# oneam/h264bsd

Measured on AMD Instinct MI355X. Metric: 1080p macroblocks/s, higher is better.
Workload: dtype u8; 1 GPU; 256 concurrent copies of test_1920x1080.h264 per GPU (73 pictures x 8160 MB), kernel-only replay from HBM-resident frame jobs, inter+intra reconstruction + in-loop deblocking; streams_per_gpu=256, parallelism=streams/1, stream_groups=1, row_bands=library default (engine.hip TailConfig)

## Files before the change

h264bsd_amd/csrc/engine.hip:

```cpp
#include <hip/hip_runtime.h>
#include <stdio.h>
#include <stdlib.h>
#include <string.h>
#include <deque>
#include <memory>
#include <mutex>
#include <vector>
#include <algorithm>
#include "kernels.hip.h"
#include "kernels/k_tensor_out.hip.h"
#include "kernels/k_tensor_aa.hip.h"
#include "kernels/k_tensor_roi.hip.h"
#include "kernels/k_tensor_remap.hip.h"
#include "kernels/k_motion.hip.h"
#include "kernels/region_common.hip.h"
#include "kernels/k_region_stats.hip.h"
#include "kernels/k_keep.hip.h"
#include "kernels/k_blend.hip.h"
#include "kernels/k_region_change.hip.h"
#include "kernels/k_region_shift.hip.h"
#include "kernels/k_cell_maps.hip.h"
#include "kernels/k_cell_boxes.hip.h"
#include "engine.h"
#include "hip_owned.h"
// ... 190 lines not shown
        Lane &l = lanes[i];
        if (g == 1 && i == 0) { l.st = e->stream; l.side = &e->side; }
        else { HIP_TRY(l.own_st.create()); l.st = l.own_st; }
        HIP_TRY(l.tail.create(hipEventDisableTiming));
        for (auto &ev : l.ring) HIP_TRY(ev.create(hipEventDisableTiming));
    }
    e->n_light = g; e->n_heavy = k;
    e->lanes.swap(lanes);
    return 0;
}

Engine *engine_get(int device = -1)
{
    if (device < 0) device = current_device();
    if (device >= MAX_DEVICES) return nullptr;
    std::lock_guard<std::mutex> lk(g_engine_mu);
    if (g_engines[device]) return g_engines[device];
    int n = 0;
    if (hipGetDeviceCount(&n) != hipSuccess || n <= 0 || device >= n) return nullptr;
    std::unique_ptr<Engine> e(new Engine());
    e->device = device;
    if (hipSetDevice(e->device) != hipSuccess || e->stream.create() != hipSuccess || e->inflight_done.create(hipEventDisableTiming) != hipSuccess ||
        ![&] {
            int lo = 0, hi = 0;
            const bool prio = hipDeviceGetStreamPriorityRange(&lo, &hi) == hipSuccess;
            return e->side.create(hi, prio);
        }() ||
        e->d_err.alloc(256) != hipSuccess || hipMemset(e->d_err, 0, 256) != hipSuccess || hipDeviceSynchronize() != hipSuccess ||
        e->h_err.alloc(64, true) != hipSuccess) return nullptr;
    e->h_err[0] = e->h_err[1] = 0;
    return g_engines[device] = e.release();
}

TailConfig g_tail;
std::mutex g_tail_mu;
TailConfig tail_config()
{
    std::lock_guard<std::mutex> lk(g_tail_mu);
    if (!g_tail.from_env) {
        g_tail.from_env = true;
        if (const char *cfg = getenv("H264BSDMI_TAIL")) {
            unsigned v[7] = { 0, 0, 0, 0, 0, 0, 0 };
            if (sscanf(cfg, "%u,%u,%u,%u,%u,%u,%u", &v[0], &v[1], &v[2], &v[3], &v[4], &v[5], &v[6]) >= 6) {
                g_tail.dbk_rows_light = v[0]; g_tail.dbk_rows_heavy = v[1]; g_tail.dbk_waves = v[2];
                g_tail.intra_rows_light = v[3]; g_tail.intra_rows_heavy = v[4]; g_tail.intra_waves = v[5];
                g_tail.dbk_chroma_waves = v[6];
            } else fprintf(stderr, "h264bsd-mi355x: H264BSDMI_TAIL=%s ignored (expected six or seven numbers)\n", cfg);
        }
        if (const char *cfg = getenv("H264BSDMI_BAND_BUDGET")) g_tail.band_budget = (uint32_t)strtoul(cfg, nullptr, 10);
        if (const char *cfg = getenv("H264BSDMI_HEAVY_BUDGET")) g_tail.heavy_budget = (uint32_t)strtoul(cfg, nullptr, 10);
    }
    return g_tail;
}
static uint16_t bands_for(uint32_t hmb, uint32_t rows)
{
    if (!rows || rows >= hmb) return 1;
    return (uint16_t)std::min<uint32_t>((hmb + rows - 1) / rows, 64u);
}

std::mutex g_ticket_mu;
auto *const g_tickets = new std::vector<std::pair<hipStream_t, DeviceMem<uint32_t>>>[MAX_DEVICES];
static uint32_t *tickets_for(hipStream_t st)
{
    int dev = 0;
    if (hipGetDevice(&dev) != hipSuccess || dev < 0 || dev >= MAX_DEVICES) return nullptr;
    std::lock_guard<std::mutex> lk(g_ticket_mu);
    for (auto &p : g_tickets[dev]) if (p.first == st) return p.second;
    DeviceMem<uint32_t> d;
    if (d.alloc(64) != hipSuccess || hipMemsetAsync(d, 0, 64, st) != hipSuccess) return nullptr;
    g_tickets[dev].emplace_back(st, std::move(d));
    return g_tickets[dev].back().second;
}
}
void tickets_release(hipStream_t st)
{
    std::lock_guard<std::mutex> lk(g_ticket_mu);
    for (int d = 0; d < MAX_DEVICES; d++)
        g_tickets[d].erase(std::remove_if(g_tickets[d].begin(), g_tickets[d].end(), [&](const auto &p) { return p.first == st; }), g_tickets[d].end());
}
namespace {
static void tickets_rezero(int dev)
{
    std::lock_guard<std::mutex> lk(g_ticket_mu);
    if (dev < 0 || dev >= MAX_DEVICES) return;
    for (auto &p : g_tickets[dev]) (void)hipMemsetAsync(p.second, 0, 64, p.first);
}


void make_desc(FrameDesc &d, const uint8_t *host_blob, const uint8_t *dev_blob, uint8_t *dev_frames, uint32_t frame_bytes,
               uint8_t *dev_dbk, TickShape *shape, uint32_t *dev_err)
{
    const FjHeader *h = reinterpret_cast<const FjHeader *>(host_blob);
    d.recs = reinterpret_cast<const FjMbRec *>(dev_blob + h->rec_off);
    d.mvx = reinterpret_cast<const int16_t *>(dev_blob + h->mvx_off);
    d.coefs = reinterpret_cast<const int16_t *>(dev_blob + h->coef_off);
    d.lvl = reinterpret_cast<const uint32_t *>(dev_blob + h->lvl_off);
    d.idx = reinterpret_cast<const uint16_t *>(dev_blob + h->idx_off);
    d.copy = reinterpret_cast<const FjCopy *>(dev_blob + h->copy_off);
    d.gen = reinterpret_cast<const FjGen *>(dev_blob + h->gen_off);
    d.n_copy = h->n_copy;
    d.n_gen = h->n_gen;
    d.n_gen_uni = h->n_gen_uniform;
    d.n_gen_quad = h->n_gen_quad;
    d.dbki = reinterpret_cast<const uint16_t *>(dev_blob + h->dbk_off);
    d.n_dbk = h->n_dbk;
    d.dbk = dev_dbk;
    d.cur = dev_frames + (size_t)h->cur_slot * frame_bytes;
    d.n_mbs = h->n_mbs;
    d.n_levels = h->n_intra_levels;
    d.wmb = h->width_mbs;
    d.wmb_magic = (uint32_t)(0x100000000ull / (h->width_mbs ? h->width_mbs : 1u)) + 1u;
    d.hmb = h->height_mbs;
    d.any_deblock = h->any_deblock;
    {
        const TailConfig tc = tail_config();
        const bool heavy = h->n_intra * 4u > h->n_mbs;
        d.heavy = heavy ? 1 : 0;
        d.dbk_bands = bands_for(h->height_mbs, heavy ? tc.dbk_rows_heavy : tc.dbk_rows_light);
        d.intra_bands = h->intra_down_deps ? 1 : bands_for(h->height_mbs, heavy ? tc.intra_rows_heavy : tc.intra_rows_light);
    }
    d.err = dev_err;
    d.conv_src = nullptr; d.conv_dst = nullptr; d.conv_fmt = 0; d.conv_pad = 0;
    for (uint32_t k = 0; k < FJ_MAX_SLOTS; k++) d.slot[k] = k < h->n_slots ? dev_frames + (size_t)k * frame_bytes : nullptr;
    if (shape) {
        shape->n_frames++;
        shape->max_mbs = std::max(shape->max_mbs, h->n_mbs);
        shape->max_copy = std::max(shape->max_copy, h->n_copy);
        shape->max_gen = std::max(shape->max_gen, h->n_gen);
        shape->max_gen_uni = std::max(shape->max_gen_uni, h->n_gen_uniform);
        shape->max_gen_quad = std::max(shape->max_gen_quad, h->n_gen_quad);
        shape->max_gen_rest = std::max(shape->max_gen_rest, h->n_gen - h->n_gen_uniform - h->n_gen_quad);
        shape->max_dbk = std::max(shape->max_dbk, h->n_dbk);
        shape->any_deblock |= h->any_deblock != 0;
        shape->max_levels = std::max(shape->max_levels, h->n_intra_levels);
        shape->max_w = std::max<uint32_t>(shape->max_w, h->width_mbs);
        shape->max_h = std::max<uint32_t>(shape->max_h, h->height_mbs);
        shape->any_tail |= h->n_intra_levels != 0 || h->any_deblock != 0;
        shape->n_heavy += d.heavy;
        if (h->any_deblock) (d.heavy ? shape->want_heavy : shape->want_light)[0] = std::max<uint32_t>((d.heavy ? shape->want_heavy : shape->want_light)[0], d.dbk_bands);
        if (h->n_intra_levels) (d.heavy ? shape->want_heavy : shape->want_light)[1] = std::max<uint32_t>((d.heavy ? shape->want_heavy : shape->want_light)[1], d.intra_bands);
        if (h->n_intra_levels && h->intra_down_deps) shape->intra_whole = true;
    }
}

struct TickTimers { Event ev[6]; Event sev[5]; bool on = false; bool copy_timed = false; unsigned mask = 31u; };

static void launch_kdbk(hipStream_t st, const FrameDesc *d_desc, const TickShape &s, uint32_t launches[5])
{
    hipLaunchKernelGGL(h264k::k_dbk, dim3((s.max_dbk + 64 * DBK_WG_WAVES - 1) / (64 * DBK_WG_WAVES), s.n_frames), dim3(64 * DBK_WG_WAVES), 0, st, d_desc);
    if (launches) launches[2]++;
}
template <int PATH> static void launch_inter(hipStream_t st, const FrameDesc *d_desc, uint32_t n_max, uint32_t n_frames)
{
    constexpr uint32_t per_wg = INTER_WG_WAVES * h264k::inter_per_wave<PATH>();
    if (n_max) hipLaunchKernelGGL(h264k::k_recon_inter<PATH>, dim3((n_max + per_wg - 1) / per_wg, n_frames), dim3(64 * INTER_WG_WAVES), 0, st, d_desc);
}
std::mutex g_tail_lds_mu;
size_t g_tail_lds[2][2][MAX_DEVICES] = {};
static int tail_prepare(hipStream_t st, int which, const BandPlan &bp, const void *fn, uint32_t **tickets)
{
    const bool banded = bp.bands > 1;
    *tickets = banded ? tickets_for(st) : nullptr;
    if (banded && !*tickets) return -1;
    int dev = 0;
    HIP_TRY(hipGetDevice(&dev));
    std::lock_guard<std::mutex> lk(g_tail_lds_mu);
    if (bp.lds > g_tail_lds[which][banded][dev]) {
        HIP_TRY(hipFuncSetAttribute(fn, hipFuncAttributeMaxDynamicSharedMemorySize, (int)bp.lds));
        g_tail_lds[which][banded][dev] = bp.lds;
    }
    return 0;
}

int launch_tick(hipStream_t st, const FrameDesc *d_desc, const TickShape &s, TickTimers *tt, uint32_t launches[5],
                unsigned stages = 7u, const SideLane *side = nullptr, unsigned long long *prof = nullptr)
{
    const bool timed = tt && tt->on;
    const unsigned tmask = timed ? tt->mask : 0u;
    auto boundary = [&](unsigned i) -> int {
        if ((((tmask << 1) | tmask) >> i) & 1u) HIP_TRY(hipEventRecord(tt->ev[i], st));
        return 0;
    };
    if (boundary(0)) return -1;
    const bool do_dbk = (stages & 4u) && s.any_deblock && s.max_dbk;
    const bool do_copy = (stages & 1u) && s.max_copy;
    const bool aside = side && side->stream && do_dbk;
    const bool copy_aside = aside && do_copy && side->copy_stream;
    if (tt) tt->copy_timed = false;
    auto launch_copy = [&](hipStream_t cs) {
        hipLaunchKernelGGL(h264k::k_copy, dim3(std::min<uint32_t>((s.max_copy + 3) / 4, COPY_WGS), s.n_frames), dim3(256), 0, cs, d_desc);
        if (launches) launches[0]++;
    };
    if (aside) {
        HIP_TRY(hipEventRecord(side->fork, st));
        HIP_TRY(hipStreamWaitEvent(side->stream, side->fork, 0));
        if (copy_aside) {
            const bool ctimed = timed && (tmask & 1u) && tt->sev[3] && tt->sev[4];
            if (tt) tt->copy_timed = ctimed;
            HIP_TRY(hipStreamWaitEvent(side->copy_stream, side->fork, 0));
            if (ctimed) HIP_TRY(hipEventRecord(tt->sev[3], side->copy_stream));
            launch_copy(side->copy_stream);
            if (ctimed) HIP_TRY(hipEventRecord(tt->sev[4], side->copy_stream));
            HIP_TRY(hipEventRecord(side->copy_join, side->copy_stream));
        }
        const bool dtimed = timed && (tmask & 4u);
        if (dtimed && tt->sev[1]) HIP_TRY(hipEventRecord(tt->sev[1], side->stream));
        launch_kdbk(side->stream, d_desc, s, launches);
        if (dtimed && tt->sev[2]) HIP_TRY(hipEventRecord(tt->sev[2], side->stream));
        HIP_TRY(hipEventRecord(side->join, side->stream));
    }
    if (do_copy && !copy_aside) launch_copy(st);
    if (boundary(1)) return -1;
    if ((stages & 1u) && s.max_gen) {
        launch_inter<0>(st, d_desc, s.max_gen_uni, s.n_frames);
        launch_inter<1>(st, d_desc, s.max_gen_quad, s.n_frames);
        launch_inter<2>(st, d_desc, s.max_gen_rest, s.n_frames);
        if (launches) launches[1]++;
    }
    if (boundary(2)) return -1;
    if (do_dbk && !aside) launch_kdbk(st, d_desc, s, launches);
    if (boundary(3)) return -1;
    const TailConfig tc = tail_config();
    if (copy_aside) HIP_TRY(hipStreamWaitEvent(st, side->copy_join, 0));
    if (s.max_levels && (stages & 2u)) {
        BandPlan bp;
        if (plan_bands(s, tc, 1, std::max<uint32_t>(1u, std::min<uint32_t>(tc.intra_waves, h264k::TAIL_WAVES)), h264k::intra_lds_bytes, false, bp)) {
            fprintf(stderr, "h264bsd-mi355x: picture of %u x %u macroblocks is too large for k_frame_intra\n", s.max_w, s.max_h); return -1;
        }
        uint32_t *tickets;
        if (tail_prepare(st, 1, bp, bp.bands > 1 ? (const void *)h264k::k_frame_intra<true> : (const void *)h264k::k_frame_intra<false>, &tickets)) return -1;
        if (bp.bands > 1) hipLaunchKernelGGL(h264k::k_frame_intra<true>, dim3(s.n_frames * bp.bands), dim3(64 * bp.waves), bp.lds, st, d_desc, prof, tickets + 2, bp.bands, bp.rows, bp.light_cap);
        else hipLaunchKernelGGL(h264k::k_frame_intra<false>, dim3(s.n_frames), dim3(64 * bp.waves), bp.lds, st, d_desc, prof, nullptr, 1u, bp.rows, 1u);
        if (launches) launches[3]++;
    }
    if (boundary(4)) return -1;
    if (aside) HIP_TRY(hipStreamWaitEvent(st, side->join, 0));
    if (s.any_deblock && (stages & 4u)) {
        BandPlan bp;
        if (plan_bands(s, tc, 0, std::max<uint32_t>(1u, std::min<uint32_t>(s.dbk_waves ? s.dbk_waves : tc.dbk_waves, h264k::DBK_WAVES)), h264k::dbk_lds_bytes, true, bp)) {
            fprintf(stderr, "h264bsd-mi355x: picture %u macroblocks wide is too large for k_frame_dbk\n", s.max_w); return -1;
        }
        const uint32_t waves = bp.waves;
        const uint32_t chroma_waves = tc.dbk_chroma_waves ? tc.dbk_chroma_waves : std::max<uint32_t>(1u, (waves * 5u + 6u) / 12u);
        const uint32_t conv_waves = !s.conv ? 0u : std::min<uint32_t>(s.conv_waves ? s.conv_waves : (uint32_t)CONV_WAVES_N, waves > chroma_waves + 1u ? waves - chroma_waves - 1u : 0u);
        uint32_t *tickets;
        if (tail_prepare(st, 0, bp, bp.bands > 1 ? (const void *)h264k::k_frame_dbk<true> : (const void *)h264k::k_frame_dbk<false>, &tickets)) return -1;
        if (bp.bands > 1) hipLaunchKernelGGL(h264k::k_frame_dbk<true>, dim3(s.n_frames * bp.bands), dim3(64 * waves), bp.lds, st, d_desc, prof, tickets, bp.bands, bp.rows, bp.light_cap, chroma_waves, conv_waves);
        else hipLaunchKernelGGL(h264k::k_frame_dbk<false>, dim3(s.n_frames), dim3(64 * waves), bp.lds, st, d_desc, prof, nullptr, 1u, bp.rows, 1u, chroma_waves, conv_waves);
        if (launches) launches[4]++;
    }
    if (s.conv && !(s.any_deblock && (stages & 4u)))
        hipLaunchKernelGGL(h264k::k_convert_rest, dim3(CONVERT_WGS, s.n_frames), dim3(256), 0, st, d_desc);
    if (boundary(5)) return -1;
    HIP_TRY(hipGetLastError());
    return 0;
}

static void fold_errors(Engine *e)
{
    const uint32_t fresh = e->h_err[0] & ~e->errors;
    if (e->h_err[1] > __atomic_load_n(&e->error_events, __ATOMIC_RELAXED)) __atomic_store_n(&e->error_events, e->h_err[1], __ATOMIC_RELAXED);
    if (fresh) {
        fprintf(stderr, "h264bsd-mi355x: DEVICE ERROR 0x%x:%s%s%s — pixels of the affected pictures are not trustworthy\n", fresh,
                (fresh & DEVERR_RESIDUAL_RANGE) ? " residual outside [-512,511] reached the kernels (host check missed it)" : "",
                (fresh & DEVERR_INTRA_SCHED) ? " k_frame_intra scheduler gave up" : "", (fresh & DEVERR_DBK_SCHED) ? " k_frame_dbk scheduler gave up" : "");
        __atomic_fetch_or(&e->errors, fresh, __ATOMIC_RELAXED);
        tickets_rezero(e->device);
    }
}
int poll_errors(Engine *e)
{
    HIP_TRY(hipMemcpyAsync(e->h_err, e->d_err, 2 * sizeof(uint32_t), hipMemcpyDeviceToHost, e->stream));
    HIP_TRY(hipStreamSynchronize(e->stream));
    fold_errors(e);
    return 0;
}

int reap_locked(Engine *e, bool wait)
{
    if (e->inflight.empty()) return 0;
    if (wait) {
        if (!e->inflight_recorded) for (auto &l : e->lanes) if (l.st) (void)hipStreamSynchronize(l.st);
        if (poll_errors(e)) return -1;
    } else if (!e->inflight_recorded || hipEventQuery(e->inflight_done) != hipSuccess) return 0;
    for (auto &f : e->inflight) {
        std::lock_guard<std::mutex> ql(f.first->qmu);
        f.first->free_bufs.push_back(std::move(f.second));
    }
    e->inflight.clear();
    return 0;
}

static void fence_unref(Engine *e, StreamCtx *s)
{
    Fence *f = s->fence;
    if (!f) return;
    s->fence = nullptr;
    if (--f->refs == 0) e->fences.push_back(f);
}
static void fence_drop(Engine *e, StreamCtx *s)
{
    if (s->fence) (void)hipEventSynchronize(s->fence->ev);
    fence_unref(e, s);
}

static void kept_drop(Engine *e, StreamCtx *s)
{
    if (!s->d_kept) return;
// ... 1296 lines not shown
```

h264bsd_amd/csrc/kernels.hip.h:

```cpp
#pragma once
#include <hip/hip_runtime.h>
#include <stdint.h>
#include "framejob.h"

#include "kernels/common.hip.h"
#include "kernels/k_dbk.hip.h"
#include "kernels/k_copy.hip.h"
#include "kernels/k_recon_inter.hip.h"
#include "kernels/convert.hip.h"
#include "kernels/tail_common.hip.h"
#include "kernels/k_frame_intra.hip.h"
#include "kernels/k_frame_dbk.hip.h"
#include "kernels/k_pixels_io.hip.h"
```

h264bsd_amd/csrc/kernels/k_recon_inter.hip.h:

```cpp
#pragma once
namespace h264k {
__device__ __forceinline__ int tap6(int a, int b, int c, int d, int e, int f) { return a - 5 * (b + e) + 20 * (c + d) + f; }

__device__ __forceinline__ void luma_window_global(const uint8_t *__restrict__ p, int wmb, int w, int h, int x, int y, uint32_t rw[6][3])
{
    if (x >= 2 && x + 9 < w && y >= 2 && y + 3 < h) {
#pragma unroll
        for (int r = 0; r < 6; r++) {
            rw[r][0] = luma4_at(p, wmb, x - 2, y - 2 + r); rw[r][1] = luma4_at(p, wmb, x + 2, y - 2 + r); rw[r][2] = luma4_at(p, wmb, x + 6, y - 2 + r);
        }
    } else {
#pragma unroll
        for (int r = 0; r < 6; r++) {
            const int yy = clip3(0, h - 1, y - 2 + r);
            uint32_t a = 0, b = 0, c = 0;
#pragma unroll
            for (int i = 0; i < 4; i++) {
                a |= (uint32_t)p[luma_at(wmb, clip3(0, w - 1, x - 2 + i), yy)] << (8 * i);
                b |= (uint32_t)p[luma_at(wmb, clip3(0, w - 1, x + 2 + i), yy)] << (8 * i);
            }
            c = (uint32_t)p[luma_at(wmb, clip3(0, w - 1, x + 6), yy)];
            rw[r][0] = a; rw[r][1] = b; rw[r][2] = c;
        }
    }
// ... 327 lines not shown
        const int e = lane - 26, pp = e >= 10, e2 = pp ? e - 10 : e;
        const int pr = is_l ? lane >> 1 : e2 >> 1, pk2 = (is_l ? lane : e2) & 1;
        uint32_t mvq[4];
        uint4 pv[4];
        bool pon[4], lfast[4], cfast[4];
#pragma unroll
        for (int q = 0; q < 4; q++) {
            mvq[q] = mvc[(q >> 1) * 8 + (q & 1) * 2];
            const int mvx = (int16_t)(mvq[q] & 0xFFFFu), mvy = (int32_t)mvq[q] >> 16;
            const H264K_GLOBAL uint8_t *ref = (const H264K_GLOBAL uint8_t *)slot_ptr(fd, (refs >> (8 * q)) & 255u);
            const int xi = mbx * 16 + 8 * (q & 1) + (mvx >> 2) - 2, yi = mby * 16 + 8 * (q >> 1) + (mvy >> 2) - 2;
            const int cxi = mbx * 8 + 4 * (q & 1) + (mvx >> 3), cyi = mby * 8 + 4 * (q >> 1) + (mvy >> 3);
            lfast[q] = xi >= 0 && xi + 13 <= W && yi >= 0 && yi + 13 <= H;
            cfast[q] = cxi >= 0 && cxi + 5 <= CW && cyi >= 0 && cyi + 5 <= CH;
            const int xs = ((xi >> 4) << 4) + 16 * pk2, cxs = ((cxi >> 3) << 3) + 8 * pk2;
            pon[q] = is_l ? (lfast[q] && xs < W) : (is_c && cfast[q] && cxs < CW);
            const size_t off = !pon[q] ? (size_t)0 : is_l ? luma_at(wmb, xs, yi + pr) : chroma_at(wmb, pp, cxs, cyi + pr);
            pv[q] = ld16g(ref + off);
        }
#pragma unroll
        for (int q = 0; q < 4; q++) {
            if (pon[q]) {
                uint32_t *d32 = reinterpret_cast<uint32_t *>(is_l ? lq + q * 13 * QW_STRIDE + pr * QW_STRIDE + 16 * pk2
                                                                  : cq + (q * 2 + pp) * 5 * QC_STRIDE + pr * QC_STRIDE + 8 * pk2);
                d32[0] = pv[q].x; d32[1] = pv[q].y;
                if (is_l) { d32[2] = pv[q].z; d32[3] = pv[q].w; }
            }
            if (!lfast[q] || !cfast[q]) {
                const int mvx = (int16_t)(mvq[q] & 0xFFFFu), mvy = (int32_t)mvq[q] >> 16;
                const uint8_t *ref = slot_ptr(fd, (refs >> (8 * q)) & 255u);
                const int xi = mbx * 16 + 8 * (q & 1) + (mvx >> 2) - 2, yi = mby * 16 + 8 * (q >> 1) + (mvy >> 2) - 2;
                const int cxi = mbx * 8 + 4 * (q & 1) + (mvx >> 3), cyi = mby * 8 + 4 * (q >> 1) + (mvy >> 3);
                if (!lfast[q] && is_l) {
                    const int xs = ((xi >> 4) << 4) + 16 * pk2, yy = clip3(0, H - 1, yi + pr);
                    uint32_t *d32 = reinterpret_cast<uint32_t *>(lq + q * 13 * QW_STRIDE + pr * QW_STRIDE + 16 * pk2);
#pragma unroll
                    for (int c = 0; c < 4; c++) {
                        uint32_t v = 0;
#pragma unroll
                        for (int i = 0; i < 4; i++) v |= (uint32_t)ref[luma_at(wmb, clip3(0, W - 1, xs + 4 * c + i), yy)] << (8 * i);
                        d32[c] = v;
                    }
                }
                if (!cfast[q] && is_c) {
                    const int cxs = ((cxi >> 3) << 3) + 8 * pk2, yy = clip3(0, CH - 1, cyi + pr);
                    uint32_t *d32 = reinterpret_cast<uint32_t *>(cq + (q * 2 + pp) * 5 * QC_STRIDE + pr * QC_STRIDE + 8 * pk2);
#pragma unroll
                    for (int c = 0; c < 2; c++) {
                        uint32_t v = 0;
#pragma unroll
                        for (int i = 0; i < 4; i++) v |= (uint32_t)ref[chroma_at(wmb, pp, clip3(0, CW - 1, cxs + 4 * c + i), yy)] << (8 * i);
                        d32[c] = v;
                    }
                }
            }
        }
        wave_sync();
        {
            const int q = (by >> 1) * 2 + (bx >> 1);
            const uint32_t mvm = q == 0 ? mvq[0] : q == 1 ? mvq[1] : q == 2 ? mvq[2] : mvq[3];
            const int mvx = (int16_t)(mvm & 0xFFFFu), mvy = (int32_t)mvm >> 16;
            const int xi = mbx * 16 + 8 * (q & 1) + (mvx >> 2) - 2;
            const int o = (xi & 15) + 4 * (bx & 1), sh = 8 * (o & 3);
            luma_pred_lds(lq + q * 13 * QW_STRIDE + (4 * (by & 1) + row) * QW_STRIDE + (o & ~3), QW_STRIDE, sh, mvx & 3, mvy & 3, pl01, pl23);
        }
        {
            const int k = (lane & 31) >> 2, plane = k >> 2, cbx = k & 1, cby = (k >> 1) & 1;
            const int q = cby * 2 + cbx;
            const uint32_t mvm = q == 0 ? mvq[0] : q == 1 ? mvq[1] : q == 2 ? mvq[2] : mvq[3];
            const int mvx = (int16_t)(mvm & 0xFFFFu), mvy = (int32_t)mvm >> 16;
            const int cxi = mbx * 8 + 4 * (q & 1) + (mvx >> 3);
            const uint8_t *s0 = cq + (q * 2 + plane) * 5 * QC_STRIDE + row * QC_STRIDE + (cxi & 7) + 2 * (lane >> 5);
            pc01 = chroma_pair_lds(s0, s0 + QC_STRIDE, mvx & 7, mvy & 7);
            pc23 = pair_from_upper_half(pc01);
        }
    } else {
        {
            const int mvx = (int16_t)(mv_mine & 0xFFFFu), mvy = (int32_t)mv_mine >> 16;
            const uint8_t *ref = slot_ptr(fd, (refs >> (8 * ((by >> 1) * 2 + (bx >> 1)))) & 255u);
            const int x = mbx * 16 + bx * 4 + (mvx >> 2), y = mby * 16 + by * 4 + row + (mvy >> 2);
            int pl[4];
            if (((mvx | mvy) & 3) == 0 && x >= 0 && x + 3 < W && y >= 0 && y < H) {
                const uint32_t v = luma4_at(ref, wmb, x, y);
                pl[0] = v & 255; pl[1] = (v >> 8) & 255; pl[2] = (v >> 16) & 255; pl[3] = v >> 24;
            } else {
                uint32_t rw[6][3];
                luma_window_global(ref, wmb, W, H, x, y, rw);
                luma_from_window(rw, mvx & 3, mvy & 3, pl);
            }
            pl01 = as_s2((uint32_t)pl[0] | ((uint32_t)pl[1] << 16)); pl23 = as_s2((uint32_t)pl[2] | ((uint32_t)pl[3] << 16));
        }
        if (lane < 32) {
            int pc[4];
            const int k = lane >> 2, plane = k >> 2, cbx = k & 1, cby = (k >> 1) & 1;
            const int cy = cby * 4 + row, cx0 = cbx * 4;
#pragma unroll
            for (int pair = 0; pair < 2; pair++) {
                const int cx = cx0 + 2 * pair;
                const int lb = (cy >> 1) * 4 + (cx >> 1);
                const int mvx = mvs[2 * lb], mvy = mvs[2 * lb + 1];
                const uint8_t *ref = slot_ptr(fd, (refs >> (8 * ((cy >> 2) * 2 + (cx >> 2)))) & 255u);
                chroma_pred2(ref, wmb, plane, CW, CH, mbx * 8 + cx + (mvx >> 3), mby * 8 + cy + (mvy >> 3), mvx & 7, mvy & 7, pc + 2 * pair);
            }
            pc01 = as_s2((uint32_t)pc[0] | ((uint32_t)pc[1] << 16)); pc23 = as_s2((uint32_t)pc[2] | ((uint32_t)pc[3] << 16));
        }
    }

    asm volatile("" :: "v"(rrows.y.x), "v"(rrows.y.y), "v"(rrows.c.x), "v"(rrows.c.y), "v"(rrows.cdc.x), "v"(rrows.cdc.y));
#ifdef H264K_INTER_PROFILE
    asm volatile("" :: "v"(pl01), "v"(pl23), "v"(pc01), "v"(pc23));
#endif
    IPROF(3);
    H264K_GLOBAL uint8_t *T = cur + (size_t)mb * TILE;
    uint32_t luma_dw, chroma_dw;
    if ((ge.coded & 0x03FFFFFFu) == 0u) {
        luma_dw = perm(as_u32(pl23), as_u32(pl01), 0x06040200u);
        chroma_dw = perm(as_u32(pc23), as_u32(pc01), 0x06040200u);
    } else if (!(ge.coded & FJ_CODED_WIDE)) {
        s2 y01, y23, c01, c23;
        mb_residual_pk(ge.coded, qp_y, qp_c, lane, rrows, y01, y23, c01, c23);
        const s2 lo = pk(0), hi = pk(255);
        const s2 l01 = pk_clip(lo, hi, pl01 + y01), l23 = pk_clip(lo, hi, pl23 + y23);
        const s2 k01 = pk_clip(lo, hi, pc01 + c01), k23 = pk_clip(lo, hi, pc23 + c23);
        luma_dw = perm(as_u32(l23), as_u32(l01), 0x06040200u);
        chroma_dw = perm(as_u32(k23), as_u32(k01), 0x06040200u);
    } else {
        int ry[4], rc[4];
        report_residual_range(fd, mb_residual_compute<false>(ge.coded, qp_y, qp_c, false, coef, lane, rrows, ry, rc), lane);
        luma_dw = pack4(clip255(pl01.x + ry[0]), clip255(pl01.y + ry[1]), clip255(pl23.x + ry[2]), clip255(pl23.y + ry[3]));
        chroma_dw = pack4(clip255(pc01.x + rc[0]), clip255(pc01.y + rc[1]), clip255(pc23.x + rc[2]), clip255(pc23.y + rc[3]));
    }
#ifdef H264K_INTER_PROFILE
    asm volatile("" :: "v"(luma_dw), "v"(chroma_dw));
#endif
    IPROF(4);
    *reinterpret_cast<H264K_GLOBAL uint32_t *>(T + (by * 4 + row) * 16 + bx * 4) = luma_dw;
    if (lane < 32) {
        const int k = lane >> 2, plane = k >> 2, cbx = k & 1, cby = (k >> 1) & 1;
        *reinterpret_cast<H264K_GLOBAL uint32_t *>(T + T_CB + plane * 64 + (cby * 4 + row) * 8 + cbx * 4) = chroma_dw;
    }
    IPROF(5);
#ifdef H264K_INTER_PROFILE
    if (PATH == 0 && lane == 0 && (blockIdx.x & 63u) == 0u) {
        unsigned long long *pc64 = reinterpret_cast<unsigned long long *>(fd.err) + 8;
        for (int k = 0; k < 5; k++) atomicAdd(pc64 + k, ipt[k + 1] - ipt[k]);
        atomicAdd(pc64 + 5, 1ull);
        atomicAdd(pc64 + 6, (ge.coded & 0x03FFFFFFu) ? 1ull : 0ull);
    }
#endif
    wave_sync();
  }
}


}
```

h264bsd_amd/srchash.py:

```python
import hashlib
import os
import re

_FILES = ("kernels.hip.h", "kernels/common.hip.h", "kernels/k_dbk.hip.h", "kernels/k_copy.hip.h", "kernels/k_recon_inter.hip.h", "kernels/convert.hip.h",
          "kernels/tail_common.hip.h", "kernels/k_frame_intra.hip.h", "kernels/k_frame_dbk.hip.h", "kernels/k_pixels_io.hip.h", "framejob.h")


def _code_only(text):
    text = re.sub(r"/\*.*?\*/", " ", text, flags=re.S)
    text = re.sub(r"//[^\n]*", " ", text)
    return re.sub(r"\s+", " ", text).strip()


def kernel_source_sha256(root):
    h = hashlib.sha256()
    for f in _FILES:
        h.update(_code_only(open(os.path.join(root, "h264bsd_amd", "csrc", f)).read()).encode())
    return h.hexdigest()
```

Before: 1.851 billion macroblocks/s.

## Add lane-per-block inter reconstruction kernel for uni-pred path with class sorting

```diff
diff --git a/h264bsd_amd/csrc/engine.hip b/h264bsd_amd/csrc/engine.hip
--- a/h264bsd_amd/csrc/engine.hip
+++ b/h264bsd_amd/csrc/engine.hip
@@ -366,8 +366,15 @@
 }
 template <int PATH> static void launch_inter(hipStream_t st, const FrameDesc *d_desc, uint32_t n_max, uint32_t n_frames)
 {
+#if INTER_LANE_BLOCKS
+    if constexpr (PATH == 0) {
+        if (n_max) hipLaunchKernelGGL(h264k::k_recon_inter_lb, dim3((n_max + INTER_LB_CHUNK - 1) / INTER_LB_CHUNK, n_frames), dim3(64), 0, st, d_desc);
+    } else
+#endif
+    {
     constexpr uint32_t per_wg = INTER_WG_WAVES * h264k::inter_per_wave<PATH>();
     if (n_max) hipLaunchKernelGGL(h264k::k_recon_inter<PATH>, dim3((n_max + per_wg - 1) / per_wg, n_frames), dim3(64 * INTER_WG_WAVES), 0, st, d_desc);
+    }
 }
 std::mutex g_tail_lds_mu;
 size_t g_tail_lds[2][2][MAX_DEVICES] = {};
diff --git a/h264bsd_amd/csrc/kernels.hip.h b/h264bsd_amd/csrc/kernels.hip.h
--- a/h264bsd_amd/csrc/kernels.hip.h
+++ b/h264bsd_amd/csrc/kernels.hip.h
@@ -6,6 +6,7 @@
 #include "kernels/common.hip.h"
 #include "kernels/k_dbk.hip.h"
 #include "kernels/k_copy.hip.h"
+#include "kernels/inter_lane_block.hip.h"
 #include "kernels/k_recon_inter.hip.h"
 #include "kernels/convert.hip.h"
 #include "kernels/tail_common.hip.h"
diff --git a/h264bsd_amd/csrc/kernels/inter_lane_block.hip.h b/h264bsd_amd/csrc/kernels/inter_lane_block.hip.h
--- /dev/null
+++ b/h264bsd_amd/csrc/kernels/inter_lane_block.hip.h
@@ -0,0 +1,187 @@
+#pragma once
+namespace h264k {
+
+constexpr uint32_t lb_sel(int c) { return 0x0C000C00u | (uint32_t)c | ((uint32_t)(c + 1) << 16); }
+#define LB_CP(row, c) as_s2((c) <= 6 ? perm((row)[1], (row)[0], lb_sel((c) <= 6 ? (c) : 0)) : perm((row)[2], (row)[1], lb_sel((c) <= 6 ? 0 : (c) - 4)))
+#define LB_RND5(x) pk_clip(pk(0), pk(255), ((x) + pk(16)) >> pk(5))
+__device__ __forceinline__ s2 lb_tap6(s2 a, s2 b, s2 c, s2 d, s2 e, s2 f) { return a + f - pk(5) * (b + e) + pk(20) * (c + d); }
+__device__ __forceinline__ int lb_dot2(s2 a, s2 b, int c)
+{
+#if defined(__HIP_DEVICE_COMPILE__)
+    return __builtin_amdgcn_sdot2(a, b, c, false);
+#else
+    return (int)a.x * b.x + (int)a.y * b.y + c;
+#endif
+}
+__device__ __forceinline__ s2 lb_avg(s2 a, s2 b) { return (a + b + pk(1)) >> pk(1); }
+__device__ __forceinline__ s2 lb_pick(bool c, s2 a, s2 b) { return as_s2(c ? as_u32(a) : as_u32(b)); }
+__device__ __forceinline__ void lb_hsum(const uint32_t row[3], s2 &h01, s2 &h23)
+{
+    const s2 c0 = LB_CP(row, 0), c1 = LB_CP(row, 1), c2 = LB_CP(row, 2), c3 = LB_CP(row, 3), c4 = LB_CP(row, 4), c5 = LB_CP(row, 5), c6 = LB_CP(row, 6), c7 = LB_CP(row, 7);
+    h01 = lb_tap6(c0, c1, c2, c3, c4, c5); h23 = lb_tap6(c2, c3, c4, c5, c6, c7);
+}
+
+__device__ __forceinline__ void lb_luma_whole(const uint32_t rw[9][3], s2 o[4][2])
+{
+#pragma unroll
+    for (int r = 0; r < 4; r++) { o[r][0] = LB_CP(rw[r + 2], 2); o[r][1] = LB_CP(rw[r + 2], 4); }
+}
+__device__ __forceinline__ void lb_luma_hor(const uint32_t rw[9][3], int fx, s2 o[4][2])
+{
+    const uint32_t q01 = lb_sel(2) + (fx == 3 ? 0x00010001u : 0u), q23 = q01 + 0x00020002u;
+    const bool quarter = fx & 1;
+#pragma unroll
+    for (int r = 0; r < 4; r++) {
+        const uint32_t *row = rw[r + 2];
+        s2 h01, h23;
+        lb_hsum(row, h01, h23);
+        h01 = LB_RND5(h01); h23 = LB_RND5(h23);
+        o[r][0] = lb_pick(quarter, lb_avg(h01, as_s2(perm(row[1], row[0], q01))), h01);
+        o[r][1] = lb_pick(quarter, lb_avg(h23, as_s2(perm(row[1], row[0], q23))), h23);
+    }
+}
+__device__ __forceinline__ void lb_luma_ver(const uint32_t rw[9][3], int fy, s2 o[4][2])
+{
+    s2 a[9][2];
+#pragma unroll
+    for (int r = 0; r < 9; r++) { a[r][0] = LB_CP(rw[r], 2); a[r][1] = LB_CP(rw[r], 4); }
+    const bool quarter = fy & 1, lower = fy == 3;
+#pragma unroll
+    for (int r = 0; r < 4; r++)
+#pragma unroll
+        for (int p = 0; p < 2; p++) {
+            const s2 v = LB_RND5(lb_tap6(a[r][p], a[r + 1][p], a[r + 2][p], a[r + 3][p], a[r + 4][p], a[r + 5][p]));
+            o[r][p] = lb_pick(quarter, lb_avg(v, lb_pick(lower, a[r + 3][p], a[r + 2][p])), v);
+        }
+}
+__device__ __forceinline__ void lb_luma_diag(const uint32_t rw[9][3], int fx, int fy, s2 o[4][2])
+{
+    const uint32_t v01 = lb_sel(2) + (fx == 3 ? 0x00010001u : 0u), v23 = v01 + 0x00020002u;
+    const bool lower = fy == 3;
+    s2 a[9][2];
+#pragma unroll
+    for (int r = 0; r < 9; r++) { a[r][0] = as_s2(perm(rw[r][1], rw[r][0], v01)); a[r][1] = as_s2(perm(rw[r][1], rw[r][0], v23)); }
+#pragma unroll
+    for (int r = 0; r < 4; r++) {
+        uint32_t row[3];
+#pragma unroll
+        for (int k = 0; k < 3; k++) row[k] = lower ? rw[r + 3][k] : rw[r + 2][k];
+        s2 h01, h23;
+        lb_hsum(row, h01, h23);
+        o[r][0] = lb_avg(LB_RND5(h01), LB_RND5(lb_tap6(a[r][0], a[r + 1][0], a[r + 2][0], a[r + 3][0], a[r + 4][0], a[r + 5][0])));
+        o[r][1] = lb_avg(LB_RND5(h23), LB_RND5(lb_tap6(a[r][1], a[r + 1][1], a[r + 2][1], a[r + 3][1], a[r + 4][1], a[r + 5][1])));
+    }
+}
+__device__ __forceinline__ void lb_luma_centre(const uint32_t rw[9][3], int fx, int fy, s2 o[4][2])
+{
+    s2 vs[4][5];
+#pragma unroll
+    for (int p = 0; p < 5; p++) {
+        s2 a[9];
+#pragma unroll
+        for (int r = 0; r < 9; r++) a[r] = LB_CP(rw[r], 2 * p);
+#pragma unroll
+        for (int r = 0; r < 4; r++) vs[r][p] = lb_tap6(a[r], a[r + 1], a[r + 2], a[r + 3], a[r + 4], a[r + 5]);
+    }
+    const bool lower = fy == 3, right = fx == 3;
+#pragma unroll
+    for (int r = 0; r < 4; r++) {
+        const s2 *vp = vs[r];
+        s2 op[4];
+#pragma unroll
+        for (int k = 0; k < 4; k++) op[k] = as_s2(perm(as_u32(vp[k + 1]), as_u32(vp[k]), 0x05040302u));
+        const s2 wa = (s2){ 1, -5 }, wb = (s2){ 20, 20 }, wc = (s2){ -5, 1 };
+        int j[4];
+#pragma unroll
+        for (int i = 0; i < 4; i++) {
+            const s2 *pp = (i & 1) ? op + (i >> 1) : vp + (i >> 1);
+            j[i] = clip255(lb_dot2(pp[0], wa, lb_dot2(pp[1], wb, lb_dot2(pp[2], wc, 512))) >> 10);
+        }
+        s2 j01 = as_s2((uint32_t)j[0] | ((uint32_t)j[1] << 16)), j23 = as_s2((uint32_t)j[2] | ((uint32_t)j[3] << 16));
+        if (fy != 2) {
+            uint32_t row[3];
+#pragma unroll
+            for (int k = 0; k < 3; k++) row[k] = lower ? rw[r + 3][k] : rw[r + 2][k];
+            s2 h01, h23;
+            lb_hsum(row, h01, h23);
+            j01 = lb_avg(j01, LB_RND5(h01)); j23 = lb_avg(j23, LB_RND5(h23));
+        } else if (fx != 2) {
+            const s2 m01 = lb_pick(right, as_s2(perm(as_u32(vp[2]), as_u32(vp[1]), 0x05040302u)), vp[1]);
+            const s2 m23 = lb_pick(right, as_s2(perm(as_u32(vp[3]), as_u32(vp[2]), 0x05040302u)), vp[2]);
+            j01 = lb_avg(j01, LB_RND5(m01)); j23 = lb_avg(j23, LB_RND5(m23));
+        }
+        o[r][0] = j01; o[r][1] = j23;
+    }
+}
+
+__device__ __forceinline__ void lb_chroma_row(uint32_t a_lo, uint32_t a_hi, uint32_t b_lo, uint32_t b_hi, s2 w00, s2 w10, s2 w01, s2 w11, s2 &o01, s2 &o23)
+{
+    const s2 p0 = as_s2(perm(a_hi, a_lo, lb_sel(0))), p1 = as_s2(perm(a_hi, a_lo, lb_sel(1))), p2 = as_s2(perm(a_hi, a_lo, lb_sel(2))), p3 = as_s2(perm(a_hi, a_lo, lb_sel(3)));
+    const s2 q0 = as_s2(perm(b_hi, b_lo, lb_sel(0))), q1 = as_s2(perm(b_hi, b_lo, lb_sel(1))), q2 = as_s2(perm(b_hi, b_lo, lb_sel(2))), q3 = as_s2(perm(b_hi, b_lo, lb_sel(3)));
+    o01 = (p0 * w00 + p1 * w10 + q0 * w01 + q1 * w11 + pk(32)) >> pk(6);
+    o23 = (p2 * w00 + p3 * w10 + q2 * w01 + q3 * w11 + pk(32)) >> pk(6);
+}
+
+__device__ __forceinline__ void lb_qp_split(int qp, int &m, int &s) { s = (qp * 43) >> 8; m = qp - 6 * s; }
+__device__ __forceinline__ int lb_chroma_dc(uint32_t lo, uint32_t hi, int i, int qp_c)
+{
+    const int c0 = (int16_t)(lo & 0xFFFFu), c1 = (int32_t)lo >> 16, c2 = (int16_t)(hi & 0xFFFFu), c3 = (int32_t)hi >> 16;
+    const int f = c0 + ((i & 1) ? -c1 : c1) + ((i & 2) ? -c2 : c2) + ((i == 1 || i == 2) ? -c3 : c3);
+    int mc, sc;
+    lb_qp_split(qp_c, mc, sc);
+    const int ls = level_scale(mc, 0);
+    return sc >= 1 ? (f * ls) << (sc - 1) : (f * ls) >> 1;
+}
+__device__ __forceinline__ void lb_residual_pk(const uint32_t y[8], const uint32_t c[8], int qp_y, int qp_c, int dc, uint32_t r[4][4])
+{
+    int my, sy, mc, sc;
+    lb_qp_split(qp_y, my, sy); lb_qp_split(qp_c, mc, sc);
+    const s2 L0 = as_s2((uint32_t)(level_scale(my, 0) << sy) | ((uint32_t)(level_scale(mc, 0) << sc) << 16));
+    const s2 L1 = as_s2((uint32_t)(level_scale(my, 1) << sy) | ((uint32_t)(level_scale(mc, 1) << sc) << 16));
+    const s2 L2 = as_s2((uint32_t)(level_scale(my, 2) << sy) | ((uint32_t)(level_scale(mc, 2) << sc) << 16));
+    typedef unsigned short us2 __attribute__((ext_vector_type(2)));
+    auto mul = [](uint32_t a, s2 b) { us2 x, z; __builtin_memcpy(&x, &a, 4); __builtin_memcpy(&z, &b, 4); x = x * z; s2 o; __builtin_memcpy(&o, &x, 4); return o; };
+    s2 f[4][4];
+#pragma unroll
+    for (int i = 0; i < 4; i++) {
+        const s2 A = (i & 1) ? L1 : L0, B = (i & 1) ? L2 : L1;
+        s2 d0 = mul(perm(c[2 * i], y[2 * i], 0x05040100u), A), d1 = mul(perm(c[2 * i], y[2 * i], 0x07060302u), B);
+        const s2 d2 = mul(perm(c[2 * i + 1], y[2 * i + 1], 0x05040100u), A), d3 = mul(perm(c[2 * i + 1], y[2 * i + 1], 0x07060302u), B);
+        if (i == 0) d0 = as_s2(perm((uint32_t)dc, as_u32(d0), 0x05040100u));
+        const s2 e0 = d0 + d2, e1 = d0 - d2, e2 = (d1 >> pk(1)) - d3, e3 = d1 + (d3 >> pk(1));
+        f[i][0] = e0 + e3; f[i][1] = e1 + e2; f[i][2] = e1 - e2; f[i][3] = e0 - e3;
+    }
+#pragma unroll
+    for (int j = 0; j < 4; j++) {
+        const s2 g0 = f[0][j] + f[2][j] + pk(32), g1 = f[0][j] - f[2][j] + pk(32);
+        const s2 g2 = (f[1][j] >> pk(1)) - f[3][j], g3 = f[1][j] + (f[3][j] >> pk(1));
+        r[0][j] = as_u32((g0 + g3) >> pk(6)); r[1][j] = as_u32((g1 + g2) >> pk(6)); r[2][j] = as_u32((g1 - g2) >> pk(6)); r[3][j] = as_u32((g0 - g3) >> pk(6));
+    }
+}
+__device__ __forceinline__ bool lb_residual_32(const uint32_t lv[8], int qp, bool use_dc, int dc, int r[4][4])
+{
+    int m, sh;
+    lb_qp_split(qp, m, sh);
+    const int ls0 = level_scale(m, 0), ls1 = level_scale(m, 1), ls2 = level_scale(m, 2);
+    int f[4][4];
+#pragma unroll
+    for (int i = 0; i < 4; i++) {
+        const int lsa = (i & 1) ? ls1 : ls0, lsb = (i & 1) ? ls2 : ls1;
+        int d0 = ((int)(int16_t)(lv[2 * i] & 0xFFFFu) * lsa) << sh, d1 = (((int32_t)lv[2 * i] >> 16) * lsb) << sh;
+        const int d2 = ((int)(int16_t)(lv[2 * i + 1] & 0xFFFFu) * lsa) << sh, d3 = (((int32_t)lv[2 * i + 1] >> 16) * lsb) << sh;
+        if (i == 0 && use_dc) d0 = dc;
+        const int e0 = d0 + d2, e1 = d0 - d2, e2 = (d1 >> 1) - d3, e3 = d1 + (d3 >> 1);
+        f[i][0] = e0 + e3; f[i][1] = e1 + e2; f[i][2] = e1 - e2; f[i][3] = e0 - e3;
+    }
+    uint32_t over = 0;
+#pragma unroll
+    for (int j = 0; j < 4; j++) {
+        const int e0 = f[0][j] + f[2][j], e1 = f[0][j] - f[2][j], e2 = (f[1][j] >> 1) - f[3][j], e3 = f[1][j] + (f[3][j] >> 1);
+        r[0][j] = (e0 + e3 + 32) >> 6; r[1][j] = (e1 + e2 + 32) >> 6; r[2][j] = (e1 - e2 + 32) >> 6; r[3][j] = (e0 - e3 + 32) >> 6;
+#pragma unroll
+        for (int i = 0; i < 4; i++) over |= (uint32_t)(r[i][j] + 512);
+    }
+    return over > 1023u;
+}
+
+}
diff --git a/h264bsd_amd/csrc/kernels/k_recon_inter.hip.h b/h264bsd_amd/csrc/kernels/k_recon_inter.hip.h
--- a/h264bsd_amd/csrc/kernels/k_recon_inter.hip.h
+++ b/h264bsd_amd/csrc/kernels/k_recon_inter.hip.h
@@ -503,5 +503,280 @@
   }
 }
 
-
-}
+#ifndef INTER_LANE_BLOCKS
+#define INTER_LANE_BLOCKS 1
+#endif
+#ifndef INTER_LB_CHUNK
+#define INTER_LB_CHUNK 32
+#endif
+#ifndef INTER_LB_OCC
+#define INTER_LB_OCC 4
+#endif
+static_assert(INTER_LB_CHUNK % 4 == 0 && INTER_LB_CHUNK >= 4 && INTER_LB_CHUNK <= 64, "INTER_LB_CHUNK");
+constexpr int LB_SLOT_LDS = 1472;
+constexpr int LB_LDS = INTER_LB_CHUNK * 16 + 4 * LB_SLOT_LDS;
+__global__ __launch_bounds__(64, INTER_LB_OCC) void k_recon_inter_lb(const FrameDesc *__restrict__ frames)
+{
+    __shared__ __attribute__((aligned(16))) uint8_t lds[LB_LDS];
+    const FrameDesc &fd = FD_REF(frames, blockIdx.y);
+#if INTER_XCD == 1
+    const uint32_t cls8 = blockIdx.x & 7u, per8 = gridDim.x >> 3, rem8 = gridDim.x & 7u;
+    const uint32_t bx_ = cls8 * per8 + (cls8 < rem8 ? cls8 : rem8) + (blockIdx.x >> 3);
+#elif INTER_XCD > 1
+    const uint32_t C_ = INTER_XCD, full_ = (gridDim.x / (8u * C_)) * (8u * C_);
+    const uint32_t b_ = blockIdx.x, o_ = b_ % (8u * C_);
+    const uint32_t bx_ = b_ >= full_ ? b_ : (b_ - o_) + (o_ & 7u) * C_ + (o_ >> 3);
+#else
+    const uint32_t bx_ = blockIdx.x;
+#endif
+    const uint32_t n_uni = fd.n_gen_uni, first = bx_ * INTER_LB_CHUNK;
+    if (first >= n_uni) return;
+    const uint32_t n_here = min(n_uni - first, (uint32_t)INTER_LB_CHUNK);
+    const int lane = threadIdx.x & 63;
+    const int wmb = fd.wmb, W = wmb * 16, H = fd.hmb * 16, CW = W >> 1, CH = H >> 1;
+    const uint32_t frame_bytes = (uint32_t)wmb * fd.hmb * (uint32_t)TILE;
+    const H264K_GLOBAL uint8_t *ref0 = (const H264K_GLOBAL uint8_t *)fd.slot[0];
+    const H264K_GLOBAL uint8_t *cf = (const H264K_GLOBAL uint8_t *)fd.coefs;
+    H264K_GLOBAL uint8_t *cur = (H264K_GLOBAL uint8_t *)fd.cur;
+
+    {
+        const bool have = (uint32_t)lane < n_here;
+        uint4 e = make_uint4(0u, 0u, 0u, 0u);
+        if (have) e = ld16g((const H264K_GLOBAL uint8_t *)fd.gen + 16u * (first + (uint32_t)lane));
+        const int fx = (int)(e.y & 3u), fy = (int)((e.y >> 16) & 3u);
+        const int cls = (fx | fy) == 0 ? 0 : fy == 0 ? 1 : fx == 0 ? 2 : (fx != 2 && fy != 2) ? 3 : 4;
+        const int bin = have ? 2 * cls + ((e.w & 0x03FFFFFFu) ? 1 : 0) : 10;
+        uint32_t rank = 0, seen = 0;
+#pragma unroll
+        for (int k = 0; k < 10; k++) {
+            const unsigned long long m = __ballot(bin == k);
+            const uint32_t before = __builtin_amdgcn_mbcnt_hi((uint32_t)(m >> 32), __builtin_amdgcn_mbcnt_lo((uint32_t)m, 0u));
+            if (bin == k) rank = seen + before;
+            seen += (uint32_t)__popcll(m);
+        }
+        if (have) *reinterpret_cast<uint4 *>(lds + 16u * rank) = e;
+        wave_sync();
+    }
+
+#define LB_FRESH() asm volatile("" : "+v"(ln), "+v"(ge.x), "+v"(ge.y), "+v"(ge.z), "+v"(ge.w))
+#define LB_LANE() const int s = ln >> 4, b = ln & 15, bx = b & 3, by = b >> 2; \
+                  uint8_t *lw = lds + INTER_LB_CHUNK * 16 + s * LB_SLOT_LDS, *lc = lw + 21 * IW_STRIDE; (void)bx; (void)by; (void)lc
+#pragma unroll 1
+    for (uint32_t g = 0; g < n_here; g += 4) {
+        int ln = lane;
+        const bool on = g + (uint32_t)(lane >> 4) < n_here;
+        uint4 ge = *reinterpret_cast<const uint4 *>(lds + 16u * (g + (uint32_t)(lane >> 4)));
+        if (!on) ge = make_uint4(0u, 0u, 0u, 0u);
+        uint32_t yl[8] = { 0u, 0u, 0u, 0u, 0u, 0u, 0u, 0u }, cl[8] = { 0u, 0u, 0u, 0u, 0u, 0u, 0u, 0u }, dcl[2] = { 0u, 0u };
+        const bool any_coded = __ballot((ge.w & 0x03FFFFFFu) != 0u) != 0ull;
+      {
+        LB_FRESH();
+        LB_LANE();
+        const uint32_t mb = ge.x & 0xFFFFu, refoff = (ge.x >> 24) * frame_bytes;
+        const int mvx = (int16_t)(ge.y & 0xFFFFu), mvy = (int32_t)ge.y >> 16;
+        const uint32_t coded = ge.w;
+        const int mby = wmb == 1 ? (int)mb : (int)__umulhi(mb, fd.wmb_magic), mbx = (int)mb - mby * wmb;
+        const int xi = mbx * 16 + (mvx >> 2) - 2, yi = mby * 16 + (mvy >> 2) - 2, xs = (xi >> 4) << 4;
+        const int cxi = mbx * 8 + (mvx >> 3), cyi = mby * 8 + (mvy >> 3), cxs = (cxi >> 3) << 3;
+        const bool lfast = on && xi >= 0 && xi + 21 <= W && yi >= 0 && yi + 21 <= H;
+        const bool cfast = on && cxi >= 0 && cxi + 9 <= CW && cyi >= 0 && cyi + 9 <= CH;
+
+        uint4 vl[4];
+        uint2 vc[3];
+        bool l_on[4], c_on[3];
+        const bool any_edge = __ballot(on && !(lfast && cfast)) != 0ull;
+#pragma unroll
+        for (int i = 0; i < 4; i++) {
+            const int p = b + 16 * i, lr = (p * 43) >> 7, lk = p - 3 * lr;
+            const int lx = clip3(0, W - 16, xs + 16 * lk), yy = clip3(0, H - 1, yi + lr);
+            l_on[i] = on && p < 63 && (lk < 2 || xi - xs >= 12);
+            const uint32_t off = refoff + (uint32_t)((yy >> 4) * wmb + (lx >> 4)) * (uint32_t)TILE + (uint32_t)((yy & 15) << 4);
+            vl[i] = ld16g(ref0 + (l_on[i] ? off : 0u));
+        }
+#pragma unroll
+        for (int i = 0; i < 3; i++) {
+            const int p = b + 16 * i, cp = p >= 18, rem = cp ? p - 18 : p, cr = rem >> 1, ck = rem & 1;
+            const int cx = clip3(0, CW - 8, cxs + 8 * ck), yy = clip3(0, CH - 1, cyi + cr);
+            c_on[i] = on && p < 36;
+            const uint32_t off = refoff + (uint32_t)((yy >> 3) * wmb + (cx >> 3)) * (uint32_t)TILE + (uint32_t)(T_CB + (cp << 6) + ((yy & 7) << 3));
+            vc[i] = ld8g(ref0 + (c_on[i] ? off : 0u));
+        }
+        if (any_coded) {
+            const int k8 = b & 7;
+            const int z = z_of(bx, by);
+            const uint32_t cidx = FJ_GEN_COEF_IDX(ge.z), nl = (uint32_t)__popc(coded & 0xFFFFu), has_cdc = (coded >> 25) & 1u;
+            const bool ybit = (coded >> z) & 1u, cbit = (coded >> (16 + k8)) & 1u;
+            const uint32_t yoff = 32u * (cidx + (uint32_t)__popc(coded & ((1u << z) - 1u)));
+            const uint32_t coff = 32u * (cidx + nl + has_cdc + (uint32_t)__popc((coded >> 16) & ((1u << k8) - 1u)));
+            const uint32_t doff = 32u * (cidx + nl) + 8u * (uint32_t)(k8 >> 2);
+            const H264K_GLOBAL uint8_t *py = ybit ? cf + yoff : ref0, *pc = cbit ? cf + coff : ref0, *pd = has_cdc ? cf + doff : ref0;
+            const uint4 y0 = ld16g(py), y1 = ld16g(py + 16), c0 = ld16g(pc), c1 = ld16g(pc + 16);
+            const uint2 d0 = ld8g(pd);
+            const uint32_t ym = ybit ? ~0u : 0u, cm = cbit ? ~0u : 0u, dm = has_cdc ? ~0u : 0u;
+            yl[0] = y0.x & ym; yl[1] = y0.y & ym; yl[2] = y0.z & ym; yl[3] = y0.w & ym; yl[4] = y1.x & ym; yl[5] = y1.y & ym; yl[6] = y1.z & ym; yl[7] = y1.w & ym;
+            cl[0] = c0.x & cm; cl[1] = c0.y & cm; cl[2] = c0.z & cm; cl[3] = c0.w & cm; cl[4] = c1.x & cm; cl[5] = c1.y & cm; cl[6] = c1.z & cm; cl[7] = c1.w & cm;
+            dcl[0] = d0.x & dm; dcl[1] = d0.y & dm;
+        }
+        if (any_edge) {
+#pragma unroll
+            for (int i = 0; i < 4; i++) {
+                const int p = b + 16 * i, lr = (p * 43) >> 7, lk = p - 3 * lr, lx = xs + 16 * lk;
+                const uint32_t first = (vl[i].x & 255u) * 0x01010101u, last = (vl[i].w >> 24) * 0x01010101u;
+                if (lx < 0) vl[i] = make_uint4(first, first, first, first);
+                else if (lx >= W) vl[i] = make_uint4(last, last, last, last);
+            }
+#pragma unroll
+            for (int i = 0; i < 3; i++) {
+                const int p = b + 16 * i, cp = p >= 18, rem = cp ? p - 18 : p, ck = rem & 1, cx = cxs + 8 * ck;
+                const uint32_t first = (vc[i].x & 255u) * 0x01010101u, last = (vc[i].y >> 24) * 0x01010101u;
+                if (cx < 0) vc[i] = make_uint2(first, first);
+                else if (cx >= CW) vc[i] = make_uint2(last, last);
+            }
+        }
+#pragma unroll
+        for (int i = 0; i < 4; i++) {
+            const int p = b + 16 * i, lr = (p * 43) >> 7, lk = p - 3 * lr;
+            if (l_on[i]) {
+                uint32_t *d32 = reinterpret_cast<uint32_t *>(lw + lr * IW_STRIDE + 16 * lk);
+                d32[0] = vl[i].x; d32[1] = vl[i].y; d32[2] = vl[i].z; d32[3] = vl[i].w;
+            }
+        }
+#pragma unroll
+        for (int i = 0; i < 3; i++) {
+            const int p = b + 16 * i, cp = p >= 18, rem = cp ? p - 18 : p, cr = rem >> 1, ck = rem & 1;
+            if (c_on[i]) {
+                uint32_t *d32 = reinterpret_cast<uint32_t *>(lc + cp * 9 * IC_STRIDE + cr * IC_STRIDE + 8 * ck);
+                d32[0] = vc[i].x; d32[1] = vc[i].y;
+            }
+        }
+        wave_sync();
+      }
+
+        s2 pl[4][2];
+#pragma unroll
+        for (int r = 0; r < 4; r++) pl[r][0] = pl[r][1] = pk(0);
+        {
+            LB_FRESH();
+            LB_LANE();
+            const int mvx = (int16_t)(ge.y & 0xFFFFu), mvy = (int32_t)ge.y >> 16;
+            const int o = (((mvx >> 2) - 2) & 15) + 4 * bx, sh = 8 * (o & 3), fx = mvx & 3, fy = mvy & 3;
+            const uint8_t *src = lw + 4 * by * IW_STRIDE + (o & ~3);
+            const int cls = !on ? -1 : (fx | fy) == 0 ? 0 : fy == 0 ? 1 : fx == 0 ? 2 : (fx != 2 && fy != 2) ? 3 : 4;
+            auto row = [&](uint32_t rw[3], int r, int nd) {
+                const uint32_t *q = reinterpret_cast<const uint32_t *>(src + r * IW_STRIDE);
+                uint32_t d[4];
+#pragma unroll
+                for (int k = 0; k < 4; k++) if (k <= nd) d[k] = q[k];
+#pragma unroll
+                for (int k = 0; k < 3; k++) rw[k] = k < nd ? (uint32_t)(((unsigned long long)d[k + 1] << 32 | d[k]) >> sh) : 0u;
+            };
+            if (cls == 0) {
+                uint32_t rw[9][3] = {};
+#pragma unroll
+                for (int r = 2; r < 6; r++) row(rw[r], r, 2);
+                lb_luma_whole(rw, pl);
+            } else if (cls == 1) {
+                uint32_t rw[9][3] = {};
+#pragma unroll
+                for (int r = 2; r < 6; r++) row(rw[r], r, 3);
+                lb_luma_hor(rw, fx, pl);
+            } else if (cls == 2) {
+                uint32_t rw[9][3] = {};
+#pragma unroll
+                for (int r = 0; r < 9; r++) row(rw[r], r, 2);
+                lb_luma_ver(rw, fy, pl);
+            } else if (cls == 3) {
+                uint32_t rw[9][3] = {};
+#pragma unroll
+                for (int r = 0; r < 9; r++) row(rw[r], r, (r >= 2 && r <= 6) ? 3 : 2);
+                lb_luma_diag(rw, fx, fy, pl);
+            } else if (cls == 4) {
+                uint32_t rw[9][3] = {};
+#pragma unroll
+                for (int r = 0; r < 9; r++) row(rw[r], r, 3);
+                lb_luma_centre(rw, fx, fy, pl);
+            }
+        }
+#define LB_CHROMA_LANE() const int k8 = b & 7, plane = k8 >> 2, cbx = k8 & 1, cby = (k8 >> 1) & 1, half = b >> 3; (void)cbx
+        s2 pc[2][2];
+        {
+            LB_FRESH();
+            LB_LANE();
+            LB_CHROMA_LANE();
+            const int mvx = (int16_t)(ge.y & 0xFFFFu), mvy = (int32_t)ge.y >> 16;
+            const int ob = ((mvx >> 3) & 7) + 4 * cbx, cfx = mvx & 7, cfy = mvy & 7;
+            const uint32_t *q = reinterpret_cast<const uint32_t *>(lc + plane * 9 * IC_STRIDE + (cby * 4 + 2 * half) * IC_STRIDE + (ob & ~3));
+            uint32_t lo[3], hi[3];
+#pragma unroll
+            for (int t = 0; t < 3; t++) {
+                const uint32_t q0 = q[5 * t], q1 = q[5 * t + 1], q2 = q[5 * t + 2];
+                lo[t] = __builtin_amdgcn_alignbyte(q1, q0, (uint32_t)(ob & 3)); hi[t] = __builtin_amdgcn_alignbyte(q2, q1, (uint32_t)(ob & 3));
+            }
+            const s2 w00 = as_s2((uint32_t)((8 - cfx) * (8 - cfy)) * 0x00010001u), w10 = as_s2((uint32_t)(cfx * (8 - cfy)) * 0x00010001u);
+            const s2 w01 = as_s2((uint32_t)((8 - cfx) * cfy) * 0x00010001u), w11 = as_s2((uint32_t)(cfx * cfy) * 0x00010001u);
+            lb_chroma_row(lo[0], hi[0], lo[1], hi[1], w00, w10, w01, w11, pc[0][0], pc[0][1]);
+            lb_chroma_row(lo[1], hi[1], lo[2], hi[2], w00, w10, w01, w11, pc[1][0], pc[1][1]);
+        }
+
+        LB_FRESH();
+        LB_LANE();
+        LB_CHROMA_LANE();
+        const uint32_t mb = ge.x & 0xFFFFu, coded = ge.w;
+        const int qp_y = (int)FJ_GEN_QP_Y(ge.z), qp_c = (int)FJ_GEN_QP_C(ge.z);
+        uint32_t ldw[4], cdw[2];
+        if (!any_coded) {
+#pragma unroll
+            for (int r = 0; r < 4; r++) ldw[r] = perm(as_u32(pl[r][1]), as_u32(pl[r][0]), 0x06040200u);
+#pragma unroll
+            for (int t = 0; t < 2; t++) cdw[t] = perm(as_u32(pc[t][1]), as_u32(pc[t][0]), 0x06040200u);
+        } else {
+            const int dc = lb_chroma_dc(dcl[0], dcl[1], k8 & 3, qp_c);
+            if (__ballot((coded & FJ_CODED_WIDE) != 0u) == 0ull) {
+                uint32_t rr[4][4];
+                lb_residual_pk(yl, cl, qp_y, qp_c, dc, rr);
+                const s2 lo = pk(0), hi = pk(255);
+#pragma unroll
+                for (int r = 0; r < 4; r++) {
+                    const s2 l01 = pk_clip(lo, hi, pl[r][0] + as_s2(perm(rr[r][1], rr[r][0], 0x05040100u)));
+                    const s2 l23 = pk_clip(lo, hi, pl[r][1] + as_s2(perm(rr[r][3], rr[r][2], 0x05040100u)));
+                    ldw[r] = perm(as_u32(l23), as_u32(l01), 0x06040200u);
+                }
+#pragma unroll
+                for (int t = 0; t < 2; t++) {
+                    const uint32_t r0 = half ? rr[2 + t][0] : rr[t][0], r1 = half ? rr[2 + t][1] : rr[t][1];
+                    const uint32_t r2 = half ? rr[2 + t][2] : rr[t][2], r3 = half ? rr[2 + t][3] : rr[t][3];
+                    const s2 k01 = pk_clip(lo, hi, pc[t][0] + as_s2(perm(r1, r0, 0x07060302u)));
+                    const s2 k23 = pk_clip(lo, hi, pc[t][1] + as_s2(perm(r3, r2, 0x07060302u)));
+                    cdw[t] = perm(as_u32(k23), as_u32(k01), 0x06040200u);
+                }
+            } else {
+                int ry[4][4], rc[4][4];
+                const bool over_y = lb_residual_32(yl, qp_y, false, 0, ry), over_c = lb_residual_32(cl, qp_c, true, dc, rc);
+                report_residual_range(fd, over_y || over_c, lane);
+#pragma unroll
+                for (int r = 0; r < 4; r++)
+                    ldw[r] = pack4(clip255(pl[r][0].x + ry[r][0]), clip255(pl[r][0].y + ry[r][1]), clip255(pl[r][1].x + ry[r][2]), clip255(pl[r][1].y + ry[r][3]));
+#pragma unroll
+                for (int t = 0; t < 2; t++) {
+                    const int c0 = half ? rc[2 + t][0] : rc[t][0], c1 = half ? rc[2 + t][1] : rc[t][1], c2 = half ? rc[2 + t][2] : rc[t][2], c3 = half ? rc[2 + t][3] : rc[t][3];
+                    cdw[t] = pack4(clip255(pc[t][0].x + c0), clip255(pc[t][0].y + c1), clip255(pc[t][1].x + c2), clip255(pc[t][1].y + c3));
+                }
+            }
+        }
+        quad_transpose4(ldw[0], ldw[1], ldw[2], ldw[3], ln);
+        const uint32_t got = (uint32_t)quad_xor1((int)((b & 1) ? cdw[0] : cdw[1]));
+        H264K_GLOBAL uint8_t *T = cur + (size_t)mb * TILE;
+        if (on) {
+            st16g(T + (4 * by + bx) * 16, make_uint4(ldw[0], ldw[1], ldw[2], ldw[3]));
+            const u32x2 v = (b & 1) ? (u32x2){ got, cdw[1] } : (u32x2){ cdw[0], got };
+            *(H264K_GLOBAL u32x2 *)(T + T_CB + plane * 64 + (cby * 4 + 2 * half + (b & 1)) * 8) = v;
+        }
+        wave_sync();
+    }
+#undef LB_FRESH
+#undef LB_LANE
+#undef LB_CHROMA_LANE
+}
+
+
+}
diff --git a/h264bsd_amd/srchash.py b/h264bsd_amd/srchash.py
--- a/h264bsd_amd/srchash.py
+++ b/h264bsd_amd/srchash.py
@@ -2,7 +2,7 @@
 import os
 import re
 
-_FILES = ("kernels.hip.h", "kernels/common.hip.h", "kernels/k_dbk.hip.h", "kernels/k_copy.hip.h", "kernels/k_recon_inter.hip.h", "kernels/convert.hip.h",
+_FILES = ("kernels.hip.h", "kernels/common.hip.h", "kernels/k_dbk.hip.h", "kernels/k_copy.hip.h", "kernels/inter_lane_block.hip.h", "kernels/k_recon_inter.hip.h", "kernels/convert.hip.h",
           "kernels/tail_common.hip.h", "kernels/k_frame_intra.hip.h", "kernels/k_frame_dbk.hip.h", "kernels/k_pixels_io.hip.h", "framejob.h")
 
 
```

Result: faster. 1.896 billion macroblocks/s (median of 6 runs) (+2.4%).
